# davidlougheed/strkit

Hardware: NVIDIA B200
Metric: read x locus repeat counts per second (higher is better)
Workload: dtype u16x2/int32

## Files before the change

include/strkit_b200.h:

```cpp
#ifndef STRKIT_B200_H
#define STRKIT_B200_H

#include <stdint.h>

#ifdef __cplusplus
extern "C" {
#endif

typedef struct strk_ctx strk_ctx;
typedef struct strk_batch strk_batch;

#define STRK_OK 0
#define STRK_ERR_ARG 1
#define STRK_ERR_CUDA 2
#define STRK_ERR_NOMEM 3
#define STRK_ERR_UNSUPPORTED 4
#define STRK_ERR_SEARCH 5

#define STRK_S1_BEG_FREE 1
#define STRK_S1_END_FREE 2
#define STRK_S2_BEG_FREE 4
#define STRK_S2_END_FREE 8
#define STRK_MODE_SG 15
#define STRK_MODE_SG_QE 2
// ... 80 lines not shown
int strk_gmm_fit_counts(strk_ctx *ctx, const double *x, const int32_t *counts, const int32_t *K, const int32_t *init,
                        int64_t n_problems, int kcap, int n_alleles, int num_bootstrap, int min_allele_reads,
                        int force_gm_filter, double expansion_ratio, int filter_factor, int n_init, double *out);

int strk_call_alleles_ploidy(strk_ctx *ctx, const int32_t *cn, const double *weights, const int64_t *read_begin,
                             int64_t n_loci, const int32_t *n_alleles, int num_bootstrap, int min_reads,
                             int min_allele_reads, int force_gm_filter, double expansion_ratio, int filter_factor,
                             int n_init, uint64_t seed, int32_t *out_i, double *out_d, int32_t *out_status,
                             double *ms_out);

int strk_gmm_fit_counts_ploidy(strk_ctx *ctx, const double *x, const int32_t *counts, const int32_t *K,
                               const int32_t *n_alleles, const int32_t *init, int64_t n_problems, int kcap,
                               int num_bootstrap, int min_allele_reads, int force_gm_filter, double expansion_ratio,
                               int filter_factor, int n_init, uint64_t seed, double *out);

int strk_gmm_fit_counts_deep(strk_ctx *ctx, const double *x, const int32_t *counts, const int32_t *K,
                             const int32_t *n_alleles, const int32_t *init, int64_t n_problems, int kcap,
                             int num_bootstrap, int min_allele_reads, int force_gm_filter, double expansion_ratio,
                             int filter_factor, int n_init, uint64_t seed, double *out);

int strk_alleles_aggregate(strk_ctx *ctx, const double *rep_means, const double *rep_weights, const double *rep_stdevs,
                           const uint8_t *rep_peaks, int64_t n_loci, int n_alleles, int num_bootstrap, int32_t *out_i,
                           double *out_d);

#define STRK_TRACE_OPEN_ON_TIE 1
#define STRK_TRACE_INS_FIRST 2
#define STRK_TRACE_END_LAST 4
int strk_realign(strk_ctx *ctx, const uint8_t *arena, uint64_t arena_bytes, const uint64_t *ref_off, const int32_t *ref_len,
                 const uint64_t *read_off, const int32_t *read_len, int64_t n, int gap_open, int gap_extend, int trace_flags,
                 int32_t *score, int32_t *end_ref, uint32_t *cigar, const uint64_t *cigar_off, int32_t *cigar_len);

int strk_measure_int_peak(strk_ctx *ctx, double out_tiops[3]);

#ifdef __cplusplus
}
#endif
#endif
```

strkit_b200/_native.py:

```python
from __future__ import annotations

import ctypes as C
import os

__all__ = ["lib", "StrkError", "check", "LIB_PATH", "build_hint"]

LIB_PATH = os.environ.get("STRKIT_B200_LIB") or os.path.join(os.path.dirname(os.path.abspath(__file__)),
                                                             "libstrkit_b200.so")
build_hint = "build it with `python -c 'import __graft_entry__ as g; g.build()'` (nvcc, sm_100a)"


class StrkError(RuntimeError):

    def __init__(self, code: int, message: str):
        super().__init__(f"strkit_b200 native error {code}: {message}")
        self.code = code


_vp = C.c_void_p
_i32, _i64, _u64 = C.c_int32, C.c_int64, C.c_uint64


def _load() -> C.CDLL:
    if not os.path.exists(LIB_PATH):
# ... 11 lines not shown
        "strk_batch_upload": (C.c_int, [_vp, _vp, _u64, _vp, _vp, _vp, _i64, _vp, _vp, _vp, _i64, C.POINTER(_vp)]),
        "strk_batch_create": (C.c_int, [_vp, C.POINTER(_vp)]),
        "strk_batch_fill": (C.c_int, [_vp, _vp, _vp, _u64, _vp, _vp, _vp, _i64, _vp, _vp, _vp, _i64]),
        "strk_batch_fill_fmt": (C.c_int, [_vp, _vp, C.c_int, _vp, _u64, _vp, _vp, _vp, _i64, _vp, _vp, _vp, _i64]),
        "strk_count_reads_fmt": (C.c_int, [_vp, C.c_int, _vp, _u64, _vp, _vp, _vp, _i64, _vp, _vp, _vp, _i64, C.c_int,
                                           C.c_int, C.c_int, C.c_int, _vp]),
        "strk_batch_run": (C.c_int, [_vp, _vp, C.c_int, C.c_int, C.c_int, C.c_int, _vp]),
        "strk_batch_download": (C.c_int, [_vp, _vp, _vp]),
        "strk_batch_free": (C.c_int, [_vp, _vp]),
        "strk_count_reads": (C.c_int, [_vp, _vp, _u64, _vp, _vp, _vp, _i64, _vp, _vp, _vp, _i64, C.c_int, C.c_int,
                                       C.c_int, C.c_int, _vp]),
        "strk_get_repeat_count": (C.c_int, [_vp, C.c_int, C.c_char_p, C.c_int, C.c_char_p, C.c_int, C.c_char_p, C.c_int,
                                            C.c_char_p, C.c_int, C.c_int, C.c_int, C.c_int, C.c_int, _vp]),
        "strk_score_tables": (C.c_int, [_vp, _vp, _u64, _vp, _vp, _vp, _vp, _vp, _i64, _vp, _vp, _i64, _vp, C.c_int,
                                        _vp]),
        "strk_ref_boundary_tables": (C.c_int, [_vp, _vp, _u64, _vp, _vp, _vp, _vp, _i64, _vp, _vp, _vp, C.c_int,
                                               _vp]),
        "strk_ref_counts": (C.c_int, [_vp, _vp, _u64, _vp, _vp, _vp, _vp, _vp, _i64, _vp, _vp, C.c_int, C.c_int, _vp]),
        "strk_call_alleles": (C.c_int, [_vp, _vp, _vp, _vp, _i64, C.c_int, C.c_int, C.c_int, C.c_int, C.c_int, C.c_double,
                                        C.c_int, C.c_int, _u64, _vp, _vp, _vp, _vp]),
        "strk_gmm_fit_counts": (C.c_int, [_vp, _vp, _vp, _vp, _vp, _i64, C.c_int, C.c_int, C.c_int, C.c_int, C.c_int,
                                          C.c_double, C.c_int, C.c_int, _vp]),
        "strk_call_alleles_ploidy": (C.c_int, [_vp, _vp, _vp, _vp, _i64, _vp, C.c_int, C.c_int, C.c_int, C.c_int,
                                               C.c_double, C.c_int, C.c_int, _u64, _vp, _vp, _vp, _vp]),
        "strk_gmm_fit_counts_ploidy": (C.c_int, [_vp, _vp, _vp, _vp, _vp, _vp, _i64, C.c_int, C.c_int, C.c_int, C.c_int,
                                                 C.c_double, C.c_int, C.c_int, _u64, _vp]),
        "strk_gmm_fit_counts_deep": (C.c_int, [_vp, _vp, _vp, _vp, _vp, _vp, _i64, C.c_int, C.c_int, C.c_int, C.c_int,
                                               C.c_double, C.c_int, C.c_int, _u64, _vp]),
        "strk_alleles_aggregate": (C.c_int, [_vp, _vp, _vp, _vp, _vp, _i64, C.c_int, C.c_int, _vp, _vp]),
        "strk_realign": (C.c_int, [_vp, _vp, _u64, _vp, _vp, _vp, _vp, _i64, C.c_int, C.c_int, C.c_int, _vp, _vp, _vp, _vp,
                                   _vp]),
        "strk_get_stats": (C.c_int, [_vp, _vp]),
        "strk_measure_int_peak": (C.c_int, [_vp, _vp]),
    }
    for name, (res, args) in sig.items():
        fn = getattr(lib_, name)
        fn.restype = res
        fn.argtypes = args
    return lib_


lib = _load()
EXPORTED = ("strk_last_error", "strk_version", "strk_device_count", "strk_init", "strk_destroy", "strk_sync", "strk_host_register",
            "strk_host_unregister", "strk_batch_upload", "strk_batch_create", "strk_batch_fill", "strk_batch_fill_fmt", "strk_count_reads_fmt", "strk_batch_run", "strk_batch_download", "strk_batch_free",
            "strk_count_reads", "strk_get_repeat_count", "strk_score_tables", "strk_ref_boundary_tables", "strk_ref_counts", "strk_call_alleles", "strk_gmm_fit_counts",
            "strk_call_alleles_ploidy", "strk_gmm_fit_counts_ploidy", "strk_gmm_fit_counts_deep", "strk_alleles_aggregate", "strk_realign", "strk_get_stats", "strk_measure_int_peak")


def check(rc: int) -> None:
    if rc != 0:
        raise StrkError(rc, lib.strk_last_error().decode("utf-8", "replace"))
```

strkit_b200/csrc/api.cu:

```cuda
#include <algorithm>
#include <chrono>
#include <cmath>
#include <cstdarg>
#include <cstdio>
#include <cstdlib>
#include <cstring>
#include <mutex>
#include <new>
#include <vector>

#include "../../include/strkit_b200.h"
#include "dp_general.cuh"
#include "dp_packed.cuh"
#include "plan.cuh"
#include "dedupe.cuh"
#include "int_peak.cuh"
#include "replay.cuh"
#include "ref_path.cuh"
#include "strk_common.cuh"

static thread_local char g_err[512] = "";

static int set_err(int code, const char *fmt, ...) {
    va_list ap;
    va_start(ap, fmt);
    vsnprintf(g_err, sizeof(g_err), fmt, ap);
    va_end(ap);
    return code;
}

#define CU(call)                                                                                          \
    do {                                                                                                  \
        cudaError_t e_ = (call);                                                                          \
// ... 94 lines not shown
    DevBuf<int> lens, start, ref_size, rc, motif_len;
    DevBuf<int> wd;
    DevBuf<int> l_off, r_off, n_off;
    DevBuf<int> ids_a, ids_b;
    DevBuf<int> tier_ids;
    DevBuf<int> lists;
    DevBuf<unsigned int> cnt;
    DevBuf<int> out;
    DevBuf<unsigned char> redo;
    std::vector<int> h_wd;
    ClassLists classes;
    std::vector<RefTier> tiers;
    void release() {
        arena.release(), seq_off.release(), motif_off.release(), lens.release(), start.release(), ref_size.release();
        rc.release(), motif_len.release(), wd.release(), l_off.release(), r_off.release(), n_off.release();
        ids_a.release(), ids_b.release(), tier_ids.release(), lists.release(), cnt.release(), out.release(), redo.release();
    }
};

enum CounterSlot : int {
    Q_GENERAL = 0,
    Q_MISS = 1,
    Q_FALLBACK = 2,
    Q_MARGIN = 3,
    Q_WIDEST = 6,
    Q_INT_PEAK = 7,
    Q_CLASS = 8,
};
static_assert(Q_FALLBACK == Q_MISS + 1 && Q_MARGIN == Q_MISS + 2, "strk_batch_run reads the three words in one copy");

struct strk_ctx {
    int device = 0;
    int n_sm = 0;
    cudaStream_t side[STRK_PK_NBIN] = {nullptr};
    cudaEvent_t side_ev[STRK_PK_NBIN] = {nullptr};
    cudaEvent_t fork_ev = nullptr;
    cudaStream_t stream = nullptr;
    cudaStream_t fill_stream = nullptr;
    int prio_hi = 0;
    ScoreConsts h_consts;
    ScoreConsts *d_consts = nullptr;
    int gap = 5, end_flags = STRK_MODE_SG, tie_flags = 0;
    DevBuf<int> scratch;
    DevBuf<FamDesc> fams;
    DevBuf<int> table;
    DevBuf<long long> table64;
    DevBuf<int> list_a, list_b, list_d;
    DevBuf<long long> list_c;
    DevBuf<int> fallback;
    DevBuf<uint4> pk_scratch;
    DevBuf<double> al_rep[3];
    DevBuf<unsigned char> al_peaks;
    RefBufs ref;
    struct strk_batch *ref_batch = nullptr;
    DevBuf<int> al_i[12];
    DevBuf<double> al_d[4];
    DevBuf<long long> al_rb;
    DevBuf<long long> al_doff;
    unsigned int *d_queue = nullptr;
    unsigned int *counter(int slot) const { return d_queue + slot; }
    double *d_acc = nullptr;
    PlanStats *d_plan = nullptr;
    unsigned int *d_bin_off = nullptr;
    cudaEvent_t ev[6] = {nullptr, nullptr, nullptr, nullptr, nullptr, nullptr};
    double stats[8] = {0, 0, 0, 0, 0, 0, 0, 0};
    struct strk_batch *reuse = nullptr;
// ... 44 lines not shown

extern "C" int strk_init(int device, const int8_t matrix[STRK_NSYM * STRK_NSYM], int gap_open, int gap_extend,
                         int end_flags, int tie_flags, strk_ctx **out) {
    if (!out || !matrix) return set_err(STRK_ERR_ARG, "strk_init: null argument");
    *out = nullptr;
    if (gap_open != gap_extend)
        return set_err(STRK_ERR_UNSUPPORTED,
                       "gap_open (%d) != gap_extend (%d): only the linear-gap case the reference uses "
                       "(indel_penalty for both, repeats.py:33) is implemented",
                       gap_open, gap_extend);
    if (gap_open < 1 || gap_open > 60) return set_err(STRK_ERR_ARG, "gap penalty %d out of range [1, 60]", gap_open);
    if (end_flags < 0 || end_flags > 15) return set_err(STRK_ERR_ARG, "end_flags %d out of range", end_flags);
    int n_dev = 0;
    cudaError_t e = cudaGetDeviceCount(&n_dev);
    if (e != cudaSuccess || n_dev == 0) {
        cudaGetLastError();
        return set_err(STRK_ERR_CUDA, "no CUDA device available (%s); strkit_b200 has no CPU fallback",
                       e == cudaSuccess ? "device count is 0" : cudaGetErrorString(e));
    }
    if (device < 0 || device >= n_dev) return set_err(STRK_ERR_ARG, "device %d out of range (%d devices)", device, n_dev);
    CU(cudaSetDevice(device));
    strk_ctx *ctx = new (std::nothrow) strk_ctx();
    if (!ctx) return set_err(STRK_ERR_NOMEM, "out of host memory");
    struct Guard {
        strk_ctx *c;
        ~Guard() {
            if (c) strk_destroy(c);
        }
    } guard{ctx};
    ctx->device = device;
    cudaDeviceProp prop;
    CU(cudaGetDeviceProperties(&prop, device));
    ctx->n_sm = prop.multiProcessorCount;
    ctx->gap = gap_open;
    ctx->end_flags = end_flags;
    ctx->tie_flags = tie_flags;
    build_lut(ctx->h_consts.lut);
    for (int a = 0; a < STRK_NSYM; ++a)
        for (int b = 0; b < STRK_NSYM; ++b) {
            int v = matrix[a * STRK_NSYM + b];
            if (v < -60 || v > 60) return set_err(STRK_ERR_ARG, "matrix entry %d out of range [-60, 60]", v);
            ctx->h_consts.smat[a * STRK_NSYM + b] = (signed char)v;
        }
    for (int b = 0; b < STRK_NSYM; ++b) {
        ctx->h_consts.smat[STRK_PAD_FREE * STRK_NSYM + b] = 0;
        ctx->h_consts.smat[STRK_PAD_PEN * STRK_NSYM + b] = (signed char)(-2 * gap_open);
    }
    ctx->h_consts.gap = gap_open;
    ctx->h_consts.end_flags = end_flags;
    {
        static const int class_code[7] = {0, 1, 2, 3, 14, 15, 16};
        int ok = 1;
        for (int b = 0; b < STRK_NSYM; ++b) {
            unsigned long long tf = 0, tb = 0;
            for (int c = 0; c < 7; ++c) {
                int v = matrix[class_code[c] * STRK_NSYM + b] + 2 * gap_open;
                if (v < 0 || v > 127) ok = 0;
                tf |= (unsigned long long)(v & 0xff) << (8 * c);
            }
            tb = tf;
            ctx->h_consts.t8f[b] = tf;
            ctx->h_consts.t8b[b] = tb;
        }
        for (int a = 0; a < STRK_NSYM; ++a)
            for (int b = 0; b < STRK_NSYM; ++b) {
                int v = matrix[a * STRK_NSYM + b] + 2 * gap_open;
// ... 177 lines not shown

static size_t general_scratch_max(strk_ctx *ctx, long long n_fams, int b_len, int rowlen) {
    size_t a = general_shape(ctx, n_fams, b_len, rowlen, false).scratch;
    if (rowlen > 2) a = std::max(a, general_shape(ctx, std::min(n_fams, lat_max(ctx)), b_len, rowlen, true).scratch);
    return a;
}

static int launch_general(strk_ctx *ctx, bool ref, const FamDesc *d_fams, const int *d_order, long long n_fams,
                          const unsigned char *d_arena, void *d_table, int b_len, int rowlen, cudaStream_t st,
                          const unsigned int *d_count = nullptr) {
    if (n_fams <= 0) return STRK_OK;
    if (d_count && n_fams > (long long)ctx->n_sm * 4) n_fams = (long long)ctx->n_sm * 4;
    if (n_fams > 0x7fffffffLL) return set_err(STRK_ERR_ARG, "too many families in one launch");
    const GenShape gs = general_shape(ctx, n_fams, b_len, rowlen, general_latency_mode(ctx, n_fams, rowlen, d_count != nullptr));
    const int grid = gs.grid, GEN_THREADS = gs.warps * 32;
    const size_t total = gs.scratch;
    if (ctx->scratch.reserve(total) != cudaSuccess) {
        cudaGetLastError();
        return set_err(STRK_ERR_NOMEM, "cannot allocate %zu bytes of DP scratch", total * sizeof(int));
    }
    unsigned int *queue = ctx->counter(Q_GENERAL);
    CU(cudaMemsetAsync(queue, 0, sizeof(unsigned int), st));
    if (ref)
        dp_general_kernel<true><<<grid, GEN_THREADS, 0, st>>>(d_fams, d_order, (int)n_fams, d_arena, ctx->d_consts,
                                                              d_table, ctx->scratch.p, rowlen, b_len, queue, d_count);
    else
        dp_general_kernel<false><<<grid, GEN_THREADS, 0, st>>>(d_fams, d_order, (int)n_fams, d_arena, ctx->d_consts,
                                                               d_table, ctx->scratch.p, rowlen, b_len, queue, d_count);
    CU(cudaGetLastError());
    ctx->stats[2] += 1;
    return STRK_OK;
}

template <int R, int L>
static int launch_packed_r(strk_ctx *ctx, const FamDesc *fams, const int *list, int n, const unsigned char *arena,
                           int *table, PackedDims dims, cudaStream_t st, int ref_mode, size_t *plan_scratch,
                           long long scratch_off) {
    constexpr int HALVES = 32 / L;
    const size_t smem = pk_smem_bytes(R, dims, L);
    {
        static std::mutex mu;
        static size_t configured[64] = {0};
        std::lock_guard<std::mutex> lock(mu);
        size_t &cur = configured[ctx->device & 63];
        if (smem > cur) {
            CU(cudaFuncSetAttribute(dp_packed_kernel<R, L>, cudaFuncAttributeMaxDynamicSharedMemorySize, (int)smem));
            cur = smem;
        }
    }
    int per_sm = 0;
    CU(cudaOccupancyMaxActiveBlocksPerMultiprocessor(&per_sm, dp_packed_kernel<R, L>, pk_warps(L) * 32, smem));
    if (per_sm < 1) return set_err(STRK_ERR_CUDA, "packed kernel R=%d L=%d does not fit an SM (%zu B shared)", R, L, smem);
    long long grid = (long long)per_sm * ctx->n_sm;
    const long long need = ((long long)n + pk_warps(L) * HALVES - 1) / (pk_warps(L) * HALVES);
    if (grid > need) grid = need;
    const size_t words = pk_scratch_words_per_unit(R, dims.w_max, L) * (size_t)grid * pk_warps(L) * HALVES;
    if (plan_scratch) {
        *plan_scratch = (words + 3) / 4;
        return STRK_OK;
    }
    if (scratch_off < 0 && ctx->pk_scratch.reserve((words + 3) / 4) != cudaSuccess) {
        cudaGetLastError();
        return set_err(STRK_ERR_NOMEM, "cannot allocate %zu bytes of capture scratch", words * 4);
    }
    unsigned int *work_counter = ctx->counter(Q_CLASS + (L == 16 ? R / 2 : R));
    CU(cudaMemsetAsync(work_counter, 0, sizeof(unsigned int), st));
    dp_packed_kernel<R, L><<<(unsigned)grid, pk_warps(L) * 32, smem, st>>>(fams, list, n, arena, ctx->d_consts, table, dims,
                                                                        ctx->pk_scratch.p + (scratch_off > 0 ? scratch_off : 0),
                                                                        ctx->fallback.p, ctx->counter(Q_FALLBACK), ref_mode,
                                                                        work_counter);
    CU(cudaGetLastError());
    ctx->stats[2] += 1;
    return STRK_OK;
}

#define PK_PAIR_RMAX 8
static int pk_lanes_for_class(int R) {
    static const int rmax = [] {
        const char *e = getenv("STRK_PK_PAIRS");
        const int v = e ? atoi(e) : PK_PAIR_RMAX;
        return v < 0 ? 0 : (v > PK_PAIR_RMAX ? PK_PAIR_RMAX : v);
    }();
    return R <= rmax ? 16 : 32;
}
static PackedDims pk_dims_for_class(int R, int max_flank, int max_m, int w_max) {
    const int L = pk_lanes_for_class(R);
    PackedDims d;
    d.colt_entries = max_flank + 2 * L;
    d.prof_words = L == 16 ? pk_prof_words(2 * R, max_m, 16) : pk_prof_words(R, max_m, 32);
    d.w_max = w_max;
    return d;
}
static size_t pk_smem_for_class(int R, const PackedDims &d) {
    return pk_lanes_for_class(R) == 16 ? pk_smem_bytes(2 * R, d, 16) : pk_smem_bytes(R, d, 32);
}

static int launch_packed(strk_ctx *ctx, int R, const FamDesc *fams, const int *list, int n, const unsigned char *arena,
                         int *table, PackedDims dims, cudaStream_t st, int ref_mode = 0, size_t *plan_scratch = nullptr,
                         long long scratch_off = -1) {
    if (pk_lanes_for_class(R) == 16) {
        switch (R) {
#define PK_CASE(N) \
    case N: return launch_packed_r<2 * N, 16>(ctx, fams, list, n, arena, table, dims, st, ref_mode, plan_scratch, scratch_off);
            PK_CASE(2) PK_CASE(3) PK_CASE(4) PK_CASE(5) PK_CASE(6) PK_CASE(7) PK_CASE(8)
#undef PK_CASE
            default: break;
        }
    }
    switch (R) {
#define PK_CASE(N) \
    case N: return launch_packed_r<N, 32>(ctx, fams, list, n, arena, table, dims, st, ref_mode, plan_scratch, scratch_off);
        PK_CASE(2) PK_CASE(3) PK_CASE(4) PK_CASE(5) PK_CASE(6) PK_CASE(7) PK_CASE(8) PK_CASE(9) PK_CASE(10) PK_CASE(11)
        PK_CASE(12) PK_CASE(13) PK_CASE(14) PK_CASE(15) PK_CASE(16)
#undef PK_CASE
        default: return set_err(STRK_ERR_ARG, "packed kernel: no instantiation for %d rows per lane", R);
    }
}

static bool pk_window_ok(const strk_ctx *ctx, int kernel, int ref_mode, int W) {
    return kernel != STRK_KERNEL_GENERAL && ctx->h_consts.packed_ok && (ref_mode ? 2 * W : W) <= PK_WINDOW_MAX;
}
static int pk_class(const strk_ctx *ctx, int kernel, int ref_mode, int W, int fl, int tr, int fr, int m) {
    return pk_window_ok(ctx, kernel, ref_mode, W) ? strk_pk_class(fl, tr, fr, m) : 0;
}

static int pk_table_w(int ref_mode, int W) { return ref_mode ? 2 * W - 1 : (W + 3) / 4 * 4; }

static int launch_pass(strk_ctx *ctx, const DpPass &p, cudaStream_t st, long long *n_packed) {
    static const long long fan_max = [] {
        const char *e = getenv("STRK_PK_FANOUT_MAX");
        return e ? atoll(e) : 131072LL;
    }();
    const bool ref = p.ref_mode != 0;
    *n_packed = 0;
    long long packed_total = 0;
    for (int k = 1; k < STRK_PK_NBIN; ++k) packed_total += p.cnt[k];
    if (!packed_total) return launch_general(ctx, ref, p.fams, p.list[0], p.cnt[0], p.arena, p.table, p.b_len, p.rowlen, st);

    PackedDims dims[STRK_PK_NBIN];
    bool fits[STRK_PK_NBIN] = {false};
    bool overlap = p.cnt[0] > 0;
    long long fams_max = std::max(p.cnt[0], std::min(packed_total, (long long)ctx->n_sm * 4));
    for (int k = 1; k < STRK_PK_NBIN; ++k) {
        if (!p.cnt[k]) continue;
        dims[k] = pk_dims_for_class(k, p.flank[k], p.mmax[k], pk_table_w(p.ref_mode, p.w[k]));
        fits[k] = pk_smem_for_class(k, dims[k]) <= 200 * 1024;
        overlap = overlap && fits[k];
        fams_max = std::max(fams_max, p.cnt[k]);
    }
    const size_t total = general_scratch_max(ctx, fams_max, p.b_len, p.rowlen);
    if (ctx->scratch.reserve(total) != cudaSuccess) {
        cudaGetLastError();
        return set_err(STRK_ERR_NOMEM, "cannot allocate %zu bytes of DP scratch", total * sizeof(int));
    }
    if (ctx->fallback.reserve((size_t)packed_total) != cudaSuccess) {
        cudaGetLastError();
        return set_err(STRK_ERR_NOMEM, "cannot allocate the fallback list");
    }
    CU(cudaMemsetAsync(ctx->counter(Q_FALLBACK), 0, sizeof(unsigned int), st));
    if (!ctx->fork_ev) CU(cudaEventCreateWithFlags(&ctx->fork_ev, cudaEventDisableTiming));
    int rc = STRK_OK;
    if (overlap) {
        if (!ctx->side[0]) CU(cudaStreamCreateWithPriority(&ctx->side[0], cudaStreamNonBlocking, ctx->prio_hi));
        if (!ctx->side_ev[0]) CU(cudaEventCreateWithFlags(&ctx->side_ev[0], cudaEventDisableTiming));
        CU(cudaEventRecord(ctx->fork_ev, st));
        CU(cudaStreamWaitEvent(ctx->side[0], ctx->fork_ev, 0));
        rc = launch_general(ctx, ref, p.fams, p.list[0], p.cnt[0], p.arena, p.table, p.b_len, p.rowlen, ctx->side[0]);
        if (rc) return rc;
        CU(cudaEventRecord(ctx->side_ev[0], ctx->side[0]));
    }
    long long fan_off[STRK_PK_NBIN];
    bool fan_out = false;
    if (p.n_slots <= fan_max) {
        size_t scratch = 0;
        int n_classes = 0;
        for (int k = STRK_PK_RMAX; k >= 1; --k) {
            if (!p.cnt[k] || !fits[k]) continue;
            size_t need = 0;
            rc = launch_packed(ctx, k, p.fams, p.list[k], (int)p.cnt[k], p.arena, (int *)p.table, dims[k], st, p.ref_mode,
                               &need);
            if (rc) return rc;
            fan_off[k] = (long long)scratch;
            scratch += need;
            ++n_classes;
        }
        if (n_classes >= 2) {
            if (ctx->pk_scratch.reserve(scratch) != cudaSuccess) {
                cudaGetLastError();
                return set_err(STRK_ERR_NOMEM, "cannot allocate %zu bytes of capture scratch", scratch * sizeof(uint4));
            }
            CU(cudaEventRecord(ctx->fork_ev, st));
            fan_out = true;
        }
    }
    for (int k = STRK_PK_RMAX; k >= 1; --k) {
        if (!p.cnt[k]) continue;
        if (!fits[k]) {
            rc = launch_general(ctx, ref, p.fams, p.list[k], p.cnt[k], p.arena, p.table, p.b_len, p.rowlen, st);
            if (rc) return rc;
            continue;
        }
        if (fan_out) {
            if (!ctx->side[k]) CU(cudaStreamCreateWithPriority(&ctx->side[k], cudaStreamNonBlocking, ctx->prio_hi));
            if (!ctx->side_ev[k]) CU(cudaEventCreateWithFlags(&ctx->side_ev[k], cudaEventDisableTiming));
            CU(cudaStreamWaitEvent(ctx->side[k], ctx->fork_ev, 0));
            rc = launch_packed(ctx, k, p.fams, p.list[k], (int)p.cnt[k], p.arena, (int *)p.table, dims[k], ctx->side[k],
                               p.ref_mode, nullptr, fan_off[k]);
            if (rc) return rc;
            CU(cudaEventRecord(ctx->side_ev[k], ctx->side[k]));
            CU(cudaStreamWaitEvent(st, ctx->side_ev[k], 0));
        } else {
            rc = launch_packed(ctx, k, p.fams, p.list[k], (int)p.cnt[k], p.arena, (int *)p.table, dims[k], st, p.ref_mode);
            if (rc) return rc;
        }
        *n_packed += p.cnt[k];
    }
    if (overlap) {
        CU(cudaStreamWaitEvent(st, ctx->side_ev[0], 0));
    } else {
        rc = launch_general(ctx, ref, p.fams, p.list[0], p.cnt[0], p.arena, p.table, p.b_len, p.rowlen, st);
        if (rc) return rc;
    }
    if (*n_packed)
        return launch_general(ctx, ref, p.fams, ctx->fallback.p, *n_packed, p.arena, p.table, p.b_len, p.rowlen, st,
                              ctx->counter(Q_FALLBACK));
    return STRK_OK;
}

static cudaError_t batch_bind(strk_batch *b, long long n_reads, long long n_loci) {
    const size_t nr = (size_t)(n_reads ? n_reads : 1), nl = (size_t)(n_loci ? n_loci : 1);
    cudaError_t e = b->seq_off.reserve(nr);
    if (e == cudaSuccess) e = b->lens.reserve(3 * nr);
    if (e == cudaSuccess) e = b->est.reserve(nr);
    if (e == cudaSuccess) e = b->read_locus.reserve(nr);
    if (e == cudaSuccess) e = b->order.reserve(nr);
    if (e == cudaSuccess) e = b->bin.reserve(nr);
    if (e == cudaSuccess) e = b->out.reserve(4 * nr);
    if (e == cudaSuccess) e = b->read_begin.reserve((size_t)n_loci + 1);
    if (e == cudaSuccess) e = b->motif_off.reserve(nl);
    if (e == cudaSuccess) e = b->motif_len.reserve(nl);
    if (e == cudaSuccess) e = b->status.reserve(nl);
    b->n_reads = n_reads;
    b->n_loci = n_loci;
    b->d_seq_off = b->seq_off.p, b->d_lens = b->lens.p, b->d_est = b->est.p, b->d_read_locus = b->read_locus.p;
    b->d_order = b->order.p, b->d_out = b->out.p, b->d_read_begin = b->read_begin.p;
// ... 291 lines not shown
        if (!h_status[(size_t)l]) continue;
        if (h_status[(size_t)l] == 2)
            return set_err(STRK_ERR_SEARCH, "locus %d: the search scored no size (max_iters = %d)", l, max_iters);
        loci.push_back(l);
        h_slot_begin.push_back((long long)h_read_ids.size());
        for (long long r = b->h_read_begin[(size_t)l]; r < b->h_read_begin[(size_t)l + 1]; ++r)
            h_read_ids.push_back((int)r);
    }
    h_locus_ids.swap(loci);
    if (ctx->list_a.reserve(h_read_ids.size()) != cudaSuccess || ctx->list_b.reserve(h_locus_ids.size()) != cudaSuccess ||
        ctx->list_c.reserve(h_slot_begin.size()) != cudaSuccess) {
        cudaGetLastError();
        return set_err(STRK_ERR_NOMEM, "cannot allocate widening lists");
    }
    CU(cudaMemcpyAsync(ctx->list_a.p, h_read_ids.data(), h_read_ids.size() * sizeof(int), cudaMemcpyHostToDevice, st));
    CU(cudaMemcpyAsync(ctx->list_b.p, h_locus_ids.data(), h_locus_ids.size() * sizeof(int), cudaMemcpyHostToDevice, st));
    CU(cudaMemcpyAsync(ctx->list_c.p, h_slot_begin.data(), h_slot_begin.size() * sizeof(long long), cudaMemcpyHostToDevice,
                       st));
    CU(cudaStreamSynchronize(st));
    return STRK_OK;
}

extern "C" int strk_batch_run(strk_ctx *ctx, strk_batch *b, int max_iters, int local_search_range, int step_size,
                              int kernel, void *stream) {
    if (!ctx || !b) return set_err(STRK_ERR_ARG, "strk_batch_run: null argument");
    if (max_iters < 0 || local_search_range < 0 || step_size < 0 || local_search_range > 1000 || step_size > 1000)
        return set_err(STRK_ERR_ARG, "strk_batch_run: bad search parameters");
    CU(cudaSetDevice(ctx->device));
    cudaStream_t st = stream ? (cudaStream_t)stream : ctx->stream;
    for (int k = 0; k < 8; ++k) ctx->stats[k] = 0;
    if (b->n_reads == 0) {
        return STRK_OK;
    }
    CU(cudaMemsetAsync(ctx->d_acc, 0, 4 * sizeof(double), st));

    int wd = local_search_range + step_size + 2;
    if (wd < 6) wd = 6;
    if (const char *env = getenv("STRK_WD")) {
        int v = atoi(env);
        if (v >= 1 && v <= 64) wd = v;
    }
    static const bool trace = getenv("STRK_RUN_TRACE") != nullptr;
    int ws = b->wide_short;
    if (const char *env = getenv("STRK_WIDE_SHORT")) ws = atoi(env) != 0;
    const int wd_cap = (STRK_MAX_WINDOW - 1) / 2 - 2;
    std::vector<int> h_read_ids, h_locus_ids;
    std::vector<long long> h_slot_begin;
    std::vector<unsigned char> h_bin;
    float ms_dp = 0.f, ms_replay = 0.f;
    double acc[2] = {0, 0};

    if (b->hint.reserve(2 * (size_t)(b->n_loci ? b->n_loci : 1)) != cudaSuccess) {
        cudaGetLastError();
        return set_err(STRK_ERR_NOMEM, "cannot allocate the window hints");
    }
    CU(cudaMemsetAsync(b->hint.p, 0, 2 * (size_t)b->n_loci * sizeof(double), st));

    for (int pass = 0;; ++pass) {
        if (wd > wd_cap) wd = wd_cap;
        const int threads = 256;
        const long long n_slots = pass ? (long long)h_read_ids.size() : b->n_reads;
        const long long n_list = pass ? (long long)h_locus_ids.size() : b->n_loci;
        const int *d_read_ids = pass ? ctx->list_a.p : nullptr, *d_locus_ids = pass ? ctx->list_b.p : nullptr;
        const long long *d_slot_begin = pass ? ctx->list_c.p : nullptr;
        const double *d_hint = pass ? b->hint.p : nullptr;
        int W = 2 * strk_read_wd(wd, 1, ws) + 1;
// ... 340 lines not shown
                     int b_len, int rowlen, int vcf_anchor_size) {
    RefBufs &d = ctx->ref;
    cudaStream_t st = ctx->stream;
    const int T = 128, WD_MAX = (STRK_MAX_WINDOW - 1) / 2;
    ref_plan1_kernel<<<(unsigned)((n + T - 1) / T), T, 0, st>>>(ids, n, d.seq_off.p, d.lens.p, d.start.p, d.wd.p, d.motif_off.p,
                                                               d.motif_len.p, 2 * wd + 1, ctx->fams.p, d_n);
    CU(cudaGetLastError());
    int rc = launch_general(ctx, true, ctx->fams.p, nullptr, n, d.arena.p, ctx->table64.p, b_len, rowlen, st, d_n);
    if (rc) return rc;
    ref_replay1_kernel<<<(unsigned)((n + T - 1) / T), T, 0, st>>>(ids, n, ctx->table64.p, ctx->fams.p, d.start.p, d.rc.p,
                                                                 d.ref_size.p, vcf_anchor_size, WD_MAX, d.wd.p, d.l_off.p,
                                                                 d.r_off.p, d.n_off.p, again, cnt, d_n);
    CU(cudaGetLastError());
    return STRK_OK;
}

static int ref_search_error(const unsigned int *cnt, const int32_t *rc_params) {
    if (cnt[2])
        return set_err(STRK_ERR_SEARCH, "strk_ref_counts: locus %lld left the widest window", (long long)(0x7fffffffu - cnt[2]));
    if (cnt[1]) {
        const long long l = (long long)(0x7fffffffu - cnt[1]);
        return set_err(STRK_ERR_SEARCH, "strk_ref_counts: locus %lld scored no size (max_iters = %d)", l, rc_params[3 * l]);
    }
    return STRK_OK;
}

extern "C" int strk_ref_counts(strk_ctx *ctx, const uint8_t *arena, uint64_t arena_bytes, const uint64_t *seq_off,
                               const int32_t *lens, const int32_t *start_count, const int32_t *ref_size,
                               const int32_t *rc_params, int64_t n_loci, const uint64_t *motif_off,
                               const int32_t *motif_len, int vcf_anchor_size, int respect_coords, int32_t *out) {
    if (!ctx || !arena || !seq_off || !lens || !start_count || !ref_size || !rc_params || !motif_off || !motif_len || !out)
        return set_err(STRK_ERR_ARG, "strk_ref_counts: null argument");
    if (n_loci <= 0 || n_loci > 0x7ffffff0LL) return set_err(STRK_ERR_ARG, "strk_ref_counts: bad locus count");
    auto now = [] { return std::chrono::duration<double, std::milli>(std::chrono::steady_clock::now().time_since_epoch()).count(); };
    const double t_begin = now();
    cudaStream_t st = ctx->stream;
    int rc = ref_setup(ctx, st, arena, arena_bytes, seq_off, lens, start_count, ref_size, rc_params, n_loci, motif_off,
                       motif_len);
    if (rc) return rc;
    RefBufs &d = ctx->ref;
    const size_t n = (size_t)n_loci;
    const bool phase1 = !respect_coords;
    const int CAP2 = 4096, WD_MAX = (STRK_MAX_WINDOW - 1) / 2, T = 128;
    const int wd1 = *std::max_element(d.h_wd.begin(), d.h_wd.end()), stride_w = 2 * wd1 + 1;
    const int wd1b = std::min(WD_MAX, 4 * wd1), stride_w2 = 2 * wd1b + 1;

    GenExtent ext = {};
    int wd2_max = 0;
    double cells1 = 0.0;
    ClassLists &lists = d.classes;
    lists.clear();
    size_t n_tiers = 0;
    for (int64_t l = 0; l < n_loci; ++l) {
        const int fl = lens[3 * l], tr = lens[3 * l + 1], fr = lens[3 * l + 2], m = motif_len[l];
        const int n1 = fl + tr + fr;
        ext.add(fl, fr, n1, m, start_count[l] + (fl + fr) / m + 1);
        if (phase1) {
            lists.add(pk_class(ctx, STRK_KERNEL_AUTO, 1, stride_w, fl, tr, fr, m), (int)l, m, fl, fr, stride_w);
            cells1 += (double)n1 * ((double)fl + fr + 2.0 * m * ((double)start_count[l] + d.h_wd[(size_t)l]));
        }
        const int32_t *p = rc_params + 3 * l;
        size_t t = 0;
        while (t < n_tiers && !std::equal(p, p + 3, d.tiers[t].rc)) ++t;
        if (t == n_tiers) {
            if (n_tiers == d.tiers.size()) d.tiers.emplace_back();
            RefTier &nt = d.tiers[n_tiers++];
// ... 243 lines not shown
```

strkit_b200/engine.py:

```python
from __future__ import annotations

import collections
import ctypes as C
import os
import threading
from concurrent.futures import ThreadPoolExecutor
from typing import Iterable, Iterator

import numpy as np

from . import _native
from ._native import check, lib
from .align_matrix import dna_matrix, indel_penalty
from .batcher import ReadBatch
from .repeat_count_params import RepeatCountParams

__all__ = ["Engine", "DeviceBatch", "default_engine", "MODE_SG", "MODE_SG_QE", "KERNEL_AUTO", "KERNEL_GENERAL"]

MODE_SG = 15
MODE_SG_QE = 2
KERNEL_AUTO = 0
KERNEL_GENERAL = 1
STAT_NAMES = ("executed_cells", "reference_cells", "kernel_launches", "dp_ms", "replay_ms", "widening_passes",
              "reads_packed_kernel", "reads_general_kernel")
# ... 156 lines not shown
    def score_tables(self, batch: ReadBatch, n_lo: np.ndarray, n_hi: np.ndarray, kernel: int = KERNEL_AUTO):
        batch.validate()
        _ascii_only(batch)
        n_lo = np.ascontiguousarray(n_lo, dtype=np.int32)
        n_hi = np.ascontiguousarray(n_hi, dtype=np.int32)
        width = (n_hi.astype(np.int64) - n_lo + 1)
        out_off = np.zeros(batch.n_reads, dtype=np.uint64)
        out_off[1:] = np.cumsum(width)[:-1]
        scores = np.empty(int(width.sum()), dtype=np.int32)
        motif_idx = np.repeat(np.arange(batch.n_loci, dtype=np.int32), np.diff(batch.read_begin)).astype(np.int32)
        check(lib.strk_score_tables(self._ctx, _p(batch.arena), batch.arena.nbytes, _p(batch.seq_off), _p(batch.lens),
                                    _p(motif_idx), _p(n_lo), _p(n_hi), batch.n_reads, _p(batch.motif_off),
                                    _p(batch.motif_len), batch.n_loci, _p(out_off), kernel, _p(scores)))
        return scores, out_off

    def ref_boundary_tables(self, batch: ReadBatch, n_lo: np.ndarray, n_hi: np.ndarray, kernel: int = KERNEL_AUTO):
        batch.validate()
        _ascii_only(batch)
        if batch.n_reads != batch.n_loci:
            raise ValueError("reference batches hold exactly one sequence per locus")
        n_lo = np.ascontiguousarray(n_lo, dtype=np.int32)
        n_hi = np.ascontiguousarray(n_hi, dtype=np.int32)
        width = (n_hi.astype(np.int64) - n_lo + 1)
        out_off = np.zeros(batch.n_loci, dtype=np.uint64)
        out_off[1:] = np.cumsum(width)[:-1]
        out = np.empty((int(width.sum()), 4), dtype=np.int32)
        check(lib.strk_ref_boundary_tables(self._ctx, _p(batch.arena), batch.arena.nbytes, _p(batch.seq_off),
                                           _p(batch.lens), _p(n_lo), _p(n_hi), batch.n_loci, _p(batch.motif_off),
                                           _p(batch.motif_len), _p(out_off), kernel, _p(out)))
        return out, out_off

    def ref_counts(self, batch: ReadBatch, start_count, ref_size, rc_params, vcf_anchor_size: int,
                   respect_coords: bool = False, out: np.ndarray | None = None) -> np.ndarray:
        batch.validate()
        _ascii_only(batch)
        start_count = np.ascontiguousarray(start_count, dtype=np.int32)
        ref_size = np.ascontiguousarray(ref_size, dtype=np.int32)
        rc = np.ascontiguousarray(rc_params, dtype=np.int32).reshape(batch.n_loci, 3)
        if out is None:
            out = np.empty((batch.n_loci, 8), dtype=np.int32)
        check(lib.strk_ref_counts(self._ctx, _p(batch.arena), batch.arena.nbytes, _p(batch.seq_off), _p(batch.lens),
                                  _p(start_count), _p(ref_size), _p(rc), batch.n_loci, _p(batch.motif_off),
                                  _p(batch.motif_len), vcf_anchor_size, int(respect_coords), _p(out)))
        return out

    def ref_counts_async(self, batch: ReadBatch, start_count, ref_size, rc_params, vcf_anchor_size: int,
                         respect_coords: bool = False, out_buf: np.ndarray | None = None):
        if getattr(self, "_ref_engs", None) is None:
            d, ef, tf, mat, go, ge = self._init_args
            self._ref_engs = [Engine(d, ef, tf, mat, go, ge)]
            self._aux_pool = ThreadPoolExecutor(max_workers=1, thread_name_prefix="strk-ref")
        ref_eng = self._ref_engs[0]

        def job():
            with ref_eng.lock:
                out = ref_eng.ref_counts(batch, start_count, ref_size, rc_params, vcf_anchor_size, respect_coords, out=out_buf)
                st = ref_eng.stats()
                ref_eng.launches += int(st["kernel_launches"])
            return out, st

        return self._aux_pool.submit(job)

    def measure_int_peak(self) -> dict[str, float]:
        s = np.zeros(3, dtype=np.float64)
        check(lib.strk_measure_int_peak(self._ctx, _p(s)))
        return {"alu_pipe": float(s[0]), "fma_pipe": float(s[1]), "dual_pipe": float(s[2])}

    def stats(self) -> dict[str, float]:
        s = np.zeros(8, dtype=np.float64)
        check(lib.strk_get_stats(self._ctx, _p(s)))
        return dict(zip(STAT_NAMES, s.tolist()))


_default: dict[tuple[int, int, int], Engine] = {}
_default_lock = threading.Lock()


def _forget_engines_after_fork() -> None:
    for eng in _default.values():
        eng._ctx = None
        eng._twin = None
        eng._stream_batch = None
    _default.clear()


if hasattr(os, "register_at_fork"):
    os.register_at_fork(after_in_child=_forget_engines_after_fork)


def default_engine(device: int = 0, end_flags: int = MODE_SG, tie_flags: int = 0) -> Engine:
    key = (device, end_flags, tie_flags)
    with _default_lock:
        eng = _default.get(key)
        if eng is None:
# ... 10 lines not shown
```

Measured before the change: 75.01 million.

## Reserve per-SM guest slot in packed read kernels when reference counting co-runs

```diff
diff --git a/include/strkit_b200.h b/include/strkit_b200.h
--- a/include/strkit_b200.h
+++ b/include/strkit_b200.h
@@ -136,6 +136,8 @@
 
 int strk_measure_int_peak(strk_ctx *ctx, double out_tiops[3]);
 
+int strk_corun_count(int device, int32_t out[2]);
+
 #ifdef __cplusplus
 }
 #endif
diff --git a/strkit_b200/_native.py b/strkit_b200/_native.py
--- a/strkit_b200/_native.py
+++ b/strkit_b200/_native.py
@@ -67,6 +67,7 @@
                                    _vp]),
         "strk_get_stats": (C.c_int, [_vp, _vp]),
         "strk_measure_int_peak": (C.c_int, [_vp, _vp]),
+        "strk_corun_count": (C.c_int, [C.c_int, _vp]),
     }
     for name, (res, args) in sig.items():
         fn = getattr(lib_, name)
@@ -79,7 +80,8 @@
 EXPORTED = ("strk_last_error", "strk_version", "strk_device_count", "strk_init", "strk_destroy", "strk_sync", "strk_host_register",
             "strk_host_unregister", "strk_batch_upload", "strk_batch_create", "strk_batch_fill", "strk_batch_fill_fmt", "strk_count_reads_fmt", "strk_batch_run", "strk_batch_download", "strk_batch_free",
             "strk_count_reads", "strk_get_repeat_count", "strk_score_tables", "strk_ref_boundary_tables", "strk_ref_counts", "strk_call_alleles", "strk_gmm_fit_counts",
-            "strk_call_alleles_ploidy", "strk_gmm_fit_counts_ploidy", "strk_gmm_fit_counts_deep", "strk_alleles_aggregate", "strk_realign", "strk_get_stats", "strk_measure_int_peak")
+            "strk_call_alleles_ploidy", "strk_gmm_fit_counts_ploidy", "strk_gmm_fit_counts_deep", "strk_alleles_aggregate", "strk_realign", "strk_get_stats", "strk_measure_int_peak",
+            "strk_corun_count")
 
 
 def check(rc: int) -> None:
diff --git a/strkit_b200/csrc/api.cu b/strkit_b200/csrc/api.cu
--- a/strkit_b200/csrc/api.cu
+++ b/strkit_b200/csrc/api.cu
@@ -1,4 +1,5 @@
 #include <algorithm>
+#include <atomic>
 #include <chrono>
 #include <cmath>
 #include <cstdarg>
@@ -159,6 +160,8 @@
 struct strk_ctx {
     int device = 0;
     int n_sm = 0;
+    int smem_reserved = 0;
+    bool in_reads = false, in_refs = false;
     cudaStream_t side[STRK_PK_NBIN] = {nullptr};
     cudaEvent_t side_ev[STRK_PK_NBIN] = {nullptr};
     cudaEvent_t fork_ev = nullptr;
@@ -269,6 +272,7 @@
     cudaDeviceProp prop;
     CU(cudaGetDeviceProperties(&prop, device));
     ctx->n_sm = prop.multiProcessorCount;
+    ctx->smem_reserved = (int)prop.reservedSharedMemPerBlock;
     ctx->gap = gap_open;
     ctx->end_flags = end_flags;
     ctx->tie_flags = tie_flags;
@@ -512,10 +516,63 @@
     return STRK_OK;
 }
 
+struct CoRun {
+    std::atomic<int> reads{0};
+    std::atomic<int> refs{0};
+    std::atomic<int> guest_regs{0}, guest_smem{0}, guest_warps{0};
+};
+static CoRun g_corun[64];
+static CoRun &corun(const strk_ctx *ctx) { return g_corun[ctx->device & 63]; }
+
+struct CoRunMark {
+    std::atomic<int> *cnt = nullptr;
+    bool *flag = nullptr;
+    CoRunMark(std::atomic<int> &c, bool &f) {
+        if (f) return;
+        f = true, flag = &f, cnt = &c;
+        c.fetch_add(1);
+    }
+    ~CoRunMark() {
+        if (!cnt) return;
+        cnt->fetch_sub(1);
+        *flag = false;
+    }
+    CoRunMark(const CoRunMark &) = delete;
+    CoRunMark &operator=(const CoRunMark &) = delete;
+};
+
+static bool corun_host(const strk_ctx *ctx) { return corun(ctx).refs.load() - (ctx->in_refs ? 1 : 0) > 0; }
+
+static void atomic_max(std::atomic<int> &a, int v) {
+    int cur = a.load();
+    while (cur < v && !a.compare_exchange_weak(cur, v)) {
+    }
+}
+
+static int cta_regs(const cudaFuncAttributes &a, int threads) { return (a.numRegs * 32 + 255) / 256 * 256 * ((threads + 31) / 32); }
+static int cta_smem(const strk_ctx *ctx, const cudaFuncAttributes &a, size_t dyn) {
+    return (int)(a.sharedSizeBytes + dyn) + ctx->smem_reserved;
+}
+
+static int guest_slot_ctas(const strk_ctx *ctx, int regs, int smem, int warps, int per_sm) {
+    const CoRun &c = corun(ctx);
+    const int gr = c.guest_regs.load(), gs = c.guest_smem.load(), gw = c.guest_warps.load();
+    auto cover = [](int need, int unit) { return need > 0 && unit > 0 ? (need + unit - 1) / unit : 1; };
+    const int g = std::max(cover(gr, regs), std::max(cover(gs, smem), cover(gw, warps)));
+    return std::min(g, per_sm - 1);
+}
+
+extern "C" int strk_corun_count(int device, int32_t out[2]) {
+    if (!out || device < 0 || device > 63) return set_err(STRK_ERR_ARG, "strk_corun_count: bad argument");
+    out[0] = g_corun[device].reads.load();
+    out[1] = g_corun[device].refs.load();
+    return STRK_OK;
+}
+
 template <int R, int L>
 static int launch_packed_r(strk_ctx *ctx, const FamDesc *fams, const int *list, int n, const unsigned char *arena,
                            int *table, PackedDims dims, cudaStream_t st, int ref_mode, size_t *plan_scratch,
-                           long long scratch_off) {
+                           long long scratch_off, bool guest_slot) {
     constexpr int HALVES = 32 / L;
     const size_t smem = pk_smem_bytes(R, dims, L);
     {
@@ -534,11 +591,30 @@
     long long grid = (long long)per_sm * ctx->n_sm;
     const long long need = ((long long)n + pk_warps(L) * HALVES - 1) / (pk_warps(L) * HALVES);
     if (grid > need) grid = need;
+    const long long full = grid;
+    int g = 0;
+    if (ctx->in_refs || guest_slot) {
+        cudaFuncAttributes fa;
+        CU(cudaFuncGetAttributes(&fa, dp_packed_kernel<R, L>));
+        const int regs = cta_regs(fa, pk_warps(L) * 32), sm = cta_smem(ctx, fa, smem);
+        if (ctx->in_refs) {
+            CoRun &c = corun(ctx);
+            atomic_max(c.guest_regs, regs), atomic_max(c.guest_smem, sm), atomic_max(c.guest_warps, pk_warps(L));
+        }
+        if (guest_slot) {
+            g = guest_slot_ctas(ctx, regs, sm, pk_warps(L), per_sm);
+            grid = std::min(grid, (long long)(per_sm - g) * ctx->n_sm);
+        }
+    }
     const size_t words = pk_scratch_words_per_unit(R, dims.w_max, L) * (size_t)grid * pk_warps(L) * HALVES;
     if (plan_scratch) {
         *plan_scratch = (words + 3) / 4;
         return STRK_OK;
     }
+    static const bool trace = getenv("STRK_RUN_TRACE") != nullptr;
+    if (trace && grid < full)
+        fprintf(stderr, "[launch_packed %p] R=%d L=%d leaves a guest slot: %lld of %lld CTAs (%d per SM, g %d)\n",
+                (void *)ctx, R, L, grid, full, per_sm, g);
     if (scratch_off < 0 && ctx->pk_scratch.reserve((words + 3) / 4) != cudaSuccess) {
         cudaGetLastError();
         return set_err(STRK_ERR_NOMEM, "cannot allocate %zu bytes of capture scratch", words * 4);
@@ -576,12 +652,12 @@
 }
 
 static int launch_packed(strk_ctx *ctx, int R, const FamDesc *fams, const int *list, int n, const unsigned char *arena,
-                         int *table, PackedDims dims, cudaStream_t st, int ref_mode = 0, size_t *plan_scratch = nullptr,
-                         long long scratch_off = -1) {
+                         int *table, PackedDims dims, cudaStream_t st, int ref_mode, size_t *plan_scratch,
+                         long long scratch_off, bool guest_slot) {
     if (pk_lanes_for_class(R) == 16) {
         switch (R) {
 #define PK_CASE(N) \
-    case N: return launch_packed_r<2 * N, 16>(ctx, fams, list, n, arena, table, dims, st, ref_mode, plan_scratch, scratch_off);
+    case N: return launch_packed_r<2 * N, 16>(ctx, fams, list, n, arena, table, dims, st, ref_mode, plan_scratch, scratch_off, guest_slot);
             PK_CASE(2) PK_CASE(3) PK_CASE(4) PK_CASE(5) PK_CASE(6) PK_CASE(7) PK_CASE(8)
 #undef PK_CASE
             default: break;
@@ -589,7 +665,7 @@
     }
     switch (R) {
 #define PK_CASE(N) \
-    case N: return launch_packed_r<N, 32>(ctx, fams, list, n, arena, table, dims, st, ref_mode, plan_scratch, scratch_off);
+    case N: return launch_packed_r<N, 32>(ctx, fams, list, n, arena, table, dims, st, ref_mode, plan_scratch, scratch_off, guest_slot);
         PK_CASE(2) PK_CASE(3) PK_CASE(4) PK_CASE(5) PK_CASE(6) PK_CASE(7) PK_CASE(8) PK_CASE(9) PK_CASE(10) PK_CASE(11)
         PK_CASE(12) PK_CASE(13) PK_CASE(14) PK_CASE(15) PK_CASE(16)
 #undef PK_CASE
@@ -649,6 +725,7 @@
         if (rc) return rc;
         CU(cudaEventRecord(ctx->side_ev[0], ctx->side[0]));
     }
+    const bool guest_slot = corun_host(ctx);
     long long fan_off[STRK_PK_NBIN];
     bool fan_out = false;
     if (p.n_slots <= fan_max) {
@@ -658,7 +735,7 @@
             if (!p.cnt[k] || !fits[k]) continue;
             size_t need = 0;
             rc = launch_packed(ctx, k, p.fams, p.list[k], (int)p.cnt[k], p.arena, (int *)p.table, dims[k], st, p.ref_mode,
-                               &need);
+                               &need, -1, guest_slot);
             if (rc) return rc;
             fan_off[k] = (long long)scratch;
             scratch += need;
@@ -685,12 +762,13 @@
             if (!ctx->side_ev[k]) CU(cudaEventCreateWithFlags(&ctx->side_ev[k], cudaEventDisableTiming));
             CU(cudaStreamWaitEvent(ctx->side[k], ctx->fork_ev, 0));
             rc = launch_packed(ctx, k, p.fams, p.list[k], (int)p.cnt[k], p.arena, (int *)p.table, dims[k], ctx->side[k],
-                               p.ref_mode, nullptr, fan_off[k]);
+                               p.ref_mode, nullptr, fan_off[k], guest_slot);
             if (rc) return rc;
             CU(cudaEventRecord(ctx->side_ev[k], ctx->side[k]));
             CU(cudaStreamWaitEvent(st, ctx->side_ev[k], 0));
         } else {
-            rc = launch_packed(ctx, k, p.fams, p.list[k], (int)p.cnt[k], p.arena, (int *)p.table, dims[k], st, p.ref_mode);
+            rc = launch_packed(ctx, k, p.fams, p.list[k], (int)p.cnt[k], p.arena, (int *)p.table, dims[k], st, p.ref_mode,
+                               nullptr, -1, guest_slot);
             if (rc) return rc;
         }
         *n_packed += p.cnt[k];
@@ -1048,6 +1126,7 @@
     if (b->n_reads == 0) {
         return STRK_OK;
     }
+    const CoRunMark mark(corun(ctx).reads, ctx->in_reads);
     CU(cudaMemsetAsync(ctx->d_acc, 0, 4 * sizeof(double), st));
 
     int wd = local_search_range + step_size + 2;
@@ -1454,6 +1533,7 @@
     if (!ctx || !arena || !seq_off || !lens || !start_count || !ref_size || !rc_params || !motif_off || !motif_len || !out)
         return set_err(STRK_ERR_ARG, "strk_ref_counts: null argument");
     if (n_loci <= 0 || n_loci > 0x7ffffff0LL) return set_err(STRK_ERR_ARG, "strk_ref_counts: bad locus count");
+    const CoRunMark mark(corun(ctx).refs, ctx->in_refs);
     auto now = [] { return std::chrono::duration<double, std::milli>(std::chrono::steady_clock::now().time_since_epoch()).count(); };
     const double t_begin = now();
     cudaStream_t st = ctx->stream;
diff --git a/strkit_b200/engine.py b/strkit_b200/engine.py
--- a/strkit_b200/engine.py
+++ b/strkit_b200/engine.py
@@ -212,6 +212,9 @@
 
     def ref_counts(self, batch: ReadBatch, start_count, ref_size, rc_params, vcf_anchor_size: int,
                    respect_coords: bool = False, out: np.ndarray | None = None) -> np.ndarray:
+        return self._ref_counts(batch, start_count, ref_size, rc_params, vcf_anchor_size, respect_coords, out)
+
+    def _ref_counts(self, batch, start_count, ref_size, rc_params, vcf_anchor_size, respect_coords, out, entering=None):
         batch.validate()
         _ascii_only(batch)
         start_count = np.ascontiguousarray(start_count, dtype=np.int32)
@@ -219,6 +222,8 @@
         rc = np.ascontiguousarray(rc_params, dtype=np.int32).reshape(batch.n_loci, 3)
         if out is None:
             out = np.empty((batch.n_loci, 8), dtype=np.int32)
+        if entering is not None:
+            entering.set()
         check(lib.strk_ref_counts(self._ctx, _p(batch.arena), batch.arena.nbytes, _p(batch.seq_off), _p(batch.lens),
                                   _p(start_count), _p(ref_size), _p(rc), batch.n_loci, _p(batch.motif_off),
                                   _p(batch.motif_len), vcf_anchor_size, int(respect_coords), _p(out)))
@@ -232,14 +237,24 @@
             self._aux_pool = ThreadPoolExecutor(max_workers=1, thread_name_prefix="strk-ref")
         ref_eng = self._ref_engs[0]
 
+        entering = threading.Event()
+
         def job():
-            with ref_eng.lock:
-                out = ref_eng.ref_counts(batch, start_count, ref_size, rc_params, vcf_anchor_size, respect_coords, out=out_buf)
-                st = ref_eng.stats()
-                ref_eng.launches += int(st["kernel_launches"])
-            return out, st
-
-        return self._aux_pool.submit(job)
+            try:
+                with ref_eng.lock:
+                    out = ref_eng._ref_counts(batch, start_count, ref_size, rc_params, vcf_anchor_size, respect_coords,
+                                              out_buf, entering)
+                    st = ref_eng.stats()
+                    ref_eng.launches += int(st["kernel_launches"])
+                return out, st
+            finally:
+                entering.set()
+
+        ahead = getattr(self, "_ref_last", None)
+        fut = self._ref_last = self._aux_pool.submit(job)
+        if ahead is None or ahead.done():
+            entering.wait()
+        return fut
 
     def measure_int_peak(self) -> dict[str, float]:
         s = np.zeros(3, dtype=np.float64)
```

New measurement: 63.32 million (median of 6 runs). 0.844x the previous value.
